# sanderslab/magellanmapper

Measured on AMD Instinct MI355X. Metric: Mvoxels/s, 2048x2048x1024 uint16 stack, 5-sigma LoG blob detection, higher is better.
Workload: dtype f16x2 MFMA (f32 accumulate) + 16-bit fixed-point intermediates; f64 re-score of every candidate

## Files before the change

### magellanmapper_amd/csrc/mmx_rescore.hip

```cpp

#include <algorithm>
#include <type_traits>

#include "mmx_common.h"

#define MMX_MAX_SIGMAS 64

struct mmx_rescore_params {
    int32_t radius[MMX_MAX_SIGMAS];
    double norm[MMX_MAX_SIGMAS];
    int32_t strip;
    int32_t n_blocks;
};

namespace {

template <typename StoreT>
__device__ __forceinline__ double corr_at(const double* vals, int st, int R, const double* w)
{
    double acc = vals[R * st] * w[0];
    for (int k = R; k >= 1; --k) acc += (vals[(R - k) * st] + vals[(R + k) * st]) * w[k];
    return (double)(StoreT)acc;
}

constexpr int kLoadRegs = 16;
constexpr int kMaxCols = 4;
template <typename InT, int NC>
struct z_cfg {
    static constexpr int raw = kLoadRegs / (2 * NC);
    static constexpr int TB = raw >= 8 ? 8 : raw >= 4 ? 4 : raw >= 2 ? 2 : 1;
};
__host__ __device__ __forceinline__ int rescore_col_class(int ncols)
{
    const int cols = (ncols + MMX_WG - 1) / MMX_WG;
    const int passes = (cols + kMaxCols - 1) / kMaxCols;
    const int per = (cols + passes - 1) / passes;
    return per <= 1 ? 1 : per <= 2 ? 2 : 4;
}

template <typename T> struct off_type { using type = T; };

template <typename InT, typename StoreT, int NC, bool INTERIOR, typename OffT>
__device__ __forceinline__ void z_phase(const InT* __restrict__ in, int nyb, int nxb, int pz, int py, int px0, int R, int N,
                                        int SW, int sw, int64_t sz, int64_t sy, int64_t sx,
                                        const int64_t* __restrict__ zr, const double* __restrict__ w0,
                                        const double* __restrict__ w2, double* __restrict__ zp0, double* __restrict__ zp2)
{
    constexpr int TB = z_cfg<InT, NC>::TB;
    const int ncols = N * sw;
    auto zoff = [&](int j) __attribute__((always_inline)) -> int64_t {
        if constexpr (INTERIOR) return (int64_t)(pz + j - R) * sz;
        else return zr[j];
    };
    constexpr bool kBytes = sizeof(OffT) == 4;
    auto ld = [&](OffT o, int64_t z) __attribute__((always_inline)) -> InT {
        if constexpr (kBytes) return *reinterpret_cast<const InT*>(reinterpret_cast<const char*>(in + z) + o);
        else return in[o + z];
    };
    for (int base = 0; base < ncols; base += MMX_WG * NC) {
        OffT off[NC];
        int at[NC];
#pragma unroll
        for (int c = 0; c < NC; ++c) {
            const int e = base + c * MMX_WG + (int)threadIdx.x;
            const int ec = e < ncols ? e : ncols - 1;
            const int dyi = ec / sw;
            const int dxi = ec - dyi * sw;
            const int yy = mmx_reflect(py + dyi - R, nyb);
            const int xx = mmx_reflect(px0 + dxi - R, nxb);
            off[c] = (OffT)(((int64_t)yy * sy + (int64_t)xx * sx) * (kBytes ? (int64_t)sizeof(InT) : 1));
            at[c] = e < ncols ? dyi * SW + dxi : -1;
        }
        double a0[NC], a2[NC];
        {
            const int64_t zc = zoff(R);
            InT ctr[NC];
#pragma unroll
            for (int c = 0; c < NC; ++c) ctr[c] = ld(off[c], zc);
#pragma unroll
            for (int c = 0; c < NC; ++c) {
                const double cv = mmx_vox<InT>::exact(ctr[c]);
                a0[c] = cv * w0[0];
                a2[c] = cv * w2[0];
            }
        }
        int k = R;
        auto batch = [&](auto nb) __attribute__((always_inline)) {
            constexpr int B = decltype(nb)::value;
            for (; k >= B; k -= B) {
                InT lo[NC][B], hi[NC][B];
                if constexpr (kBytes) {
#pragma unroll
                    for (int c = 0; c < NC; ++c) asm volatile("" : "+v"(off[c]));
                }
#pragma unroll
                for (int j = 0; j < B; ++j) {
                    const int64_t zl = zoff(R - (k - j)), zh = zoff(R + (k - j));
#pragma unroll
                    for (int c = 0; c < NC; ++c) {
                        lo[c][j] = ld(off[c], zl);
                        hi[c][j] = ld(off[c], zh);
                    }
                }
#pragma unroll
                for (int c = 0; c < NC; ++c) {
#pragma unroll
                    for (int j = 0; j < B; ++j) {
                        const double p = mmx_vox<InT>::exact(lo[c][j]) + mmx_vox<InT>::exact(hi[c][j]);
                        a0[c] += p * w0[k - j];
                        a2[c] += p * w2[k - j];
                    }
                }
            }
        };
        batch(std::integral_constant<int, TB>{});
        if constexpr (TB > 4) batch(std::integral_constant<int, 4>{});
        if constexpr (TB > 2) batch(std::integral_constant<int, 2>{});
        if constexpr (TB > 1) batch(std::integral_constant<int, 1>{});
#pragma unroll
        for (int c = 0; c < NC; ++c) {
            if (at[c] >= 0) {
                zp0[at[c]] = (double)(StoreT)a0[c];
                zp2[at[c]] = (double)(StoreT)a2[c];
            }
        }
    }
}

template <typename InT, typename StoreT>
__global__ void __launch_bounds__(MMX_WG)
rescore_kernel(const InT* __restrict__ vol, int64_t sz, int64_t sy, int64_t sx,
               const mmx_block* __restrict__ blocks, mmx_cand* __restrict__ pts, uint32_t cap,
               const uint32_t* __restrict__ count, const double* __restrict__ w0_tab,
               const double* __restrict__ w2_tab, mmx_rescore_params prm)
{
    extern __shared__ double smem[];
    uint32_t n = cap;
    if (count) { const uint32_t c = *count; n = c < cap ? c : cap; }
    for (uint64_t idx64 = blockIdx.x; idx64 < n; idx64 += gridDim.x) {
    const uint32_t idx = (uint32_t)idx64;
    const mmx_cand ptv = pts[idx];
    mmx_cand pt;
    pt.slot = __builtin_amdgcn_readfirstlane(ptv.slot);
    pt.s = __builtin_amdgcn_readfirstlane(ptv.s);
    pt.z = __builtin_amdgcn_readfirstlane(ptv.z);
    pt.y = __builtin_amdgcn_readfirstlane(ptv.y);
    pt.x = __builtin_amdgcn_readfirstlane(ptv.x);
    if (pt.slot < 0 || pt.slot >= prm.n_blocks || pt.s < 0 || pt.s >= MMX_MAX_SIGMAS) continue;
    const mmx_block bd = blocks[pt.slot];
    const int R = prm.radius[pt.s];
    const int N = 2 * R + 1;
    const int SW = prm.strip < N ? prm.strip : N;
    const double* w0 = w0_tab + (int64_t)pt.s * (MMX_MAX_RADIUS_GENERIC + 1);
    const double* w2 = w2_tab + (int64_t)pt.s * (MMX_MAX_RADIUS_GENERIC + 1);
    const InT* in = vol + bd.src_off;

    double* zp0 = smem;
    double* zp2 = zp0 + (size_t)N * SW;
    double* yp = zp2 + (size_t)N * SW;
    int64_t* zr = (int64_t*)(yp + 3 * (size_t)N);

    const bool interior = pt.z - R >= 0 && pt.z + R < bd.nz;
    const int cls = rescore_col_class(N * SW);
    const bool small = ((int64_t)(bd.ny - 1) * sy + (int64_t)(bd.nx - 1) * sx) * (int64_t)sizeof(InT) < (1ll << 31)
                       && sy >= 0 && sx >= 0;
    __syncthreads();
    if (!interior) {
        for (int k = threadIdx.x; k < N; k += MMX_WG) zr[k] = (int64_t)mmx_reflect(pt.z + k - R, bd.nz) * sz;
        __syncthreads();
    }
    for (int dx0 = 0; dx0 < N; dx0 += SW) {
        const int sw = (N - dx0) < SW ? (N - dx0) : SW;
        auto zrun = [&](auto nc, auto ot) __attribute__((always_inline)) {
            constexpr int NC = decltype(nc)::value;
            using OffT = typename decltype(ot)::type;
            if (interior)
                z_phase<InT, StoreT, NC, true, OffT>(in, bd.ny, bd.nx, pt.z, pt.y, pt.x + dx0, R, N, SW, sw, sz, sy, sx,
                                                     zr, w0, w2, zp0, zp2);
            else
                z_phase<InT, StoreT, NC, false, OffT>(in, bd.ny, bd.nx, pt.z, pt.y, pt.x + dx0, R, N, SW, sw, sz, sy, sx,
                                                      zr, w0, w2, zp0, zp2);
        };
        if (!small) zrun(std::integral_constant<int, 2>{}, off_type<int64_t>{});
        else switch (cls) {
            case 1: zrun(std::integral_constant<int, 1>{}, off_type<uint32_t>{}); break;
            case 2: zrun(std::integral_constant<int, 2>{}, off_type<uint32_t>{}); break;
            default: zrun(std::integral_constant<int, 4>{}, off_type<uint32_t>{}); break;
        }
        __syncthreads();
        for (int t = threadIdx.x; t < 3 * sw; t += MMX_WG) {
            const int term = t / sw;
            const int dxi = t - term * sw;
            const double* src = (term == 0 ? zp2 : zp0) + dxi;
            yp[term * N + dx0 + dxi] = corr_at<StoreT>(src, SW, R, term == 1 ? w2 : w0);
        }
        __syncthreads();
    }
    if (threadIdx.x < 3)
        zp0[threadIdx.x] = corr_at<StoreT>(yp + threadIdx.x * N, 1, R, threadIdx.x == 2 ? w2 : w0);
    __syncthreads();
    if (threadIdx.x == 0) {
        const StoreT t0 = (StoreT)zp0[0];
        const StoreT t1 = (StoreT)zp0[1];
        const StoreT t2 = (StoreT)zp0[2];
        StoreT sum = t0;
        sum += t1;
        sum += t2;
        const StoreT cube = (-sum) * (StoreT)prm.norm[pt.s];
        pts[idx].v64 = (double)cube;
    }
    }
}

template <typename InT, typename StoreT>
int launch(const mmx_volume* vol, const mmx_block* d_blocks, mmx_cand* d_pts, uint32_t cap,
           const uint32_t* d_count, const double* d_w0, const double* d_w2,
           const mmx_rescore_params& prm, size_t lds, hipStream_t s)
{
    const uint32_t gx = cap < 8192u ? cap : 8192u;
    hipLaunchKernelGGL((rescore_kernel<InT, StoreT>), dim3(gx), dim3(MMX_WG), lds, s,
                       (const InT*)vol->d_data, vol->stride_z, vol->stride_y, vol->stride_x, d_blocks,
                       d_pts, cap, d_count, d_w0, d_w2, prm);
    return hipGetLastError() == hipSuccess ? MMX_OK : MMX_ERR_HIP;
}

}

namespace {
__global__ void __launch_bounds__(MMX_WG)
expand_probes_kernel(mmx_cand* __restrict__ tab, uint32_t cap, uint32_t* __restrict__ count,
                     const uint32_t* __restrict__ n_cands, const mmx_block* __restrict__ blocks, int n_blocks, int ns)
{
    const uint32_t n = *n_cands < cap ? *n_cands : cap;
    for (uint64_t i = (uint64_t)blockIdx.x * MMX_WG + threadIdx.x; i < n; i += (uint64_t)gridDim.x * MMX_WG) {
        const mmx_cand c = tab[i];
        if (!(c.flags & MMX_CAND_CONTESTED) || c.slot < 0 || c.slot >= n_blocks) continue;
        const mmx_block bd = blocks[c.slot];
        const bool banded = (c.flags & MMX_CAND_BAND) != 0;
        int j = 0;
        for (int ds = -1; ds <= 1; ++ds)
            for (int dz = -1; dz <= 1; ++dz)
                for (int dy = -1; dy <= 1; ++dy)
                    for (int dx = -1; dx <= 1; ++dx) {
                        if ((ds | dz | dy | dx) == 0) continue;
                        const int bit = j++;
                        const int ss = c.s + ds, zz = c.z + dz, yy = c.y + dy, xx = c.x + dx;
                        if (ss < 0 || ss >= ns || zz < 0 || zz >= bd.nz || yy < 0 || yy >= bd.ny || xx < 0 || xx >= bd.nx)
                            continue;
                        if (banded && !(bit < 64 ? (c.band >> bit) & 1ull : (c.flags >> (16 + bit - 64)) & 1u)) continue;
                        const uint32_t pos = atomicAdd(count, 1u);
                        if (pos < cap) {
                            mmx_cand r;
                            r.slot = c.slot; r.s = ss; r.z = zz; r.y = yy; r.x = xx;
                            r.flags = MMX_CAND_PROBE;
                            r.v = 0.f; r.nbr_max = 0.f;
                            r.v64 = __longlong_as_double(0x7ff8000000000000LL);
                            r.band = i;
                            tab[pos] = r;
                        }
                    }
    }
}
}

extern "C" int mmx_expand_probes(mmx_cand* d_cands, uint32_t cap, uint32_t* d_count, uint32_t* d_n_cands,
                                 const mmx_block* d_blocks, int n_blocks, int n_sigma, void* stream)
{
    if (!d_cands || !d_count || !d_n_cands || !d_blocks || n_blocks < 1 || n_sigma < 1) return MMX_ERR_ARG;
    hipStream_t s = (hipStream_t)stream;
    if (hipMemcpyAsync(d_n_cands, d_count, sizeof(uint32_t), hipMemcpyDeviceToDevice, s) != hipSuccess) return MMX_ERR_HIP;
    if (cap == 0) return MMX_OK;
    mmx_timed_scope ts(MMX_K_RESCORE, s);
    const uint32_t gx = std::min<uint32_t>(1024u, (cap + MMX_WG - 1) / MMX_WG);
    hipLaunchKernelGGL(expand_probes_kernel, dim3(gx), dim3(MMX_WG), 0, s, d_cands, cap, d_count, d_n_cands, d_blocks,
                       n_blocks, n_sigma);
    return hipGetLastError() == hipSuccess ? MMX_OK : MMX_ERR_HIP;
}

extern "C" int mmx_rescore_f64(const mmx_volume* vol, const mmx_block* d_blocks, int n_blocks,
                               mmx_cand* d_pts, uint32_t cap, const uint32_t* d_count,
                               const double* d_w0, const double* d_w2, const int32_t* h_radius,
                               const double* h_norm, int n_sigma, int store_f32, void* stream)
{
    if (!vol || !vol->d_data || !d_blocks || !d_pts || !d_w0 || !d_w2 || !h_radius || !h_norm)
        return MMX_ERR_ARG;
    if (n_sigma < 1 || n_sigma > MMX_MAX_SIGMAS || n_blocks < 1) return MMX_ERR_ARG;
    if (cap == 0) return MMX_OK;
    mmx_rescore_params prm;
    int rmax = 0;
    for (int i = 0; i < MMX_MAX_SIGMAS; ++i) { prm.radius[i] = 0; prm.norm[i] = 0.0; }
    for (int i = 0; i < n_sigma; ++i) {
        if (h_radius[i] < 0 || h_radius[i] > MMX_MAX_RADIUS_GENERIC) return MMX_ERR_UNSUPPORTED;
        prm.radius[i] = h_radius[i];
        prm.norm[i] = h_norm[i];
        if (h_radius[i] > rmax) rmax = h_radius[i];
    }
    prm.n_blocks = n_blocks;
    const int N = 2 * rmax + 1;
    const size_t budget = 60 * 1024;
    const size_t fixed = (size_t)3 * N * sizeof(double) + (size_t)N * sizeof(int64_t) + 16;
    int strip = (int)((budget - fixed) / ((size_t)2 * N * sizeof(double)));
    if (strip < 1) return MMX_ERR_UNSUPPORTED;
    if (strip > N) strip = N;
    prm.strip = strip;
    const size_t lds = (size_t)2 * N * strip * sizeof(double) + fixed;
    hipStream_t s = (hipStream_t)stream;
    const bool f32s = store_f32 != 0;
    mmx_timed_scope ts(MMX_K_RESCORE, s);
    return mmx_for_voxel<MMX_VOX_ALL>(vol->dtype, MMX_ERR_ARG, [&](auto t) {
        using T = MMX_TAG_T(t);
        if constexpr (std::is_same<T, float>::value)
            if (f32s) return launch<T, float>(vol, d_blocks, d_pts, cap, d_count, d_w0, d_w2, prm, lds, s);
        return launch<T, double>(vol, d_blocks, d_pts, cap, d_count, d_w0, d_w2, prm, lds, s);
    });
}
```

### magellanmapper_amd/csrc/mmx_ymfma.hip

```cpp

#include <type_traits>

#include <cstdlib>

#include "mmx_device.h"

struct ym_cfg {
    float w2[MMX_MAX_RADIUS_FAST + 1];
    float w0[MMX_MAX_RADIUS_FAST + 1];
    float unscale;
    float start;
    float lo, eps;
    int radius;
    int reverse;
};

namespace {

#ifndef YM5_OCC
#define YM5_OCC 2
#endif
#ifndef YM6_WAVES
#define YM6_WAVES 4
#define YM6_JH 4
#define YM6_NF 4
#endif
template <int NB, bool MASK>
__global__ void __launch_bounds__(NB <= 4 ? 256 : YM6_WAVES * 64, NB <= 4 ? 3 : (YM6_WAVES == 4 ? YM5_OCC : 1))
ym_kernel(const mmx_block* __restrict__ blocks, int64_t slot_elems, int64_t tile_stride,
          const unsigned* __restrict__ gt, float* __restrict__ out, ym_cfg cfg,
          unsigned long long* __restrict__ mask)
{
    constexpr int RB = 8 * (NB - 2);
    constexpr int NF = NB <= 4 ? 4 : YM6_NF;
    __shared__ v4u frag[NB * NF * 64];
    constexpr int WAVES = NB <= 4 ? 4 : YM6_WAVES;
    constexpr int JH = NB <= 4 ? 4 : YM6_JH;
    __shared__ float tr[WAVES * 2 * 1024];

    const mmx_block bd = blocks[cfg.reverse ? gridDim.y - 1 - blockIdx.y : blockIdx.y];
    const int ntx = (bd.nx + 15) >> 4, ntz = (bd.nz + 15) >> 4;
    if ((int)blockIdx.x * (WAVES / 4) >= ntx * ntz) return;
    for (int e = threadIdx.x; e < NB * NF * 64; e += WAVES * 64) {
        const int ln = e & 63, f = e >> 6;
        const int piece = (f % NF) % (NF / 2), kern = (f % NF) / (NF / 2), t = f / NF;
        const int m = ln & 15, kq = ln >> 4;
        const int delta = RB - 16 * t;
        unsigned pk[4];
#pragma unroll
        for (int i = 0; i < 8; i += 2) {
            float v[2];
#pragma unroll
            for (int u = 0; u < 2; ++u) {
                int d = 8 * kq + i + u - m + delta;
                d = d < 0 ? -d : d;
                const float ws = d <= cfg.radius ? (kern ? cfg.w0[d] : cfg.w2[d]) : 0.f;
                const float h = (float)(_Float16)ws;
                v[u] = piece == 0 ? h : (piece == 1 ? (ws - h) * 256.f : h * 256.f);
            }
            pk[i >> 1] = pack_h2(v[0], v[1]);
        }
        frag[e] = (v4u){pk[0], pk[1], pk[2], pk[3]};
    }
    __syncthreads();

    const int wv = __builtin_amdgcn_readfirstlane((int)(threadIdx.x >> 6));
    const int tile = (int)blockIdx.x * (WAVES / 4) + (wv >> 2);
    if (tile >= ntx * ntz) return;
    const int c = tile / ntz, U = tile - c * ntz;
    const int zq = wv & 3;
    if (16 * U + 4 * zq >= bd.nz) return;
    const int lane = threadIdx.x & 63;
    const int n = bd.ny;
    const float nms_lo = cfg.lo, nms_eps = cfg.eps, us = cfg.unscale;
    const int kq = lane >> 4, n16 = lane & 15;
    const unsigned trow_b = (unsigned)(ntx * ntz) * 1024u;
    const rsrc_t rs = make_rsrc(gt + (int64_t)bd.slot * tile_stride + (int64_t)tile * 256);
    const unsigned voff = (unsigned)(zq * 256 + n16 * 16);
    const unsigned voff_s = voff + (unsigned)(8 * kq) * trow_b;
    const int xi = lane & 15;
    const int z = 16 * U + 4 * zq + (lane >> 4), x = 16 * c + xi;
    const bool real = z < bd.nz && x < bd.nx;
    float* w1 = out + (int64_t)bd.slot * slot_elems;
    const rsrc_t rsw = make_rsrc(w1);
    const unsigned ooff = (unsigned)((real ? z : 0) * bd.ny * bd.px + (real ? x : 0)) * 4u;
    const unsigned row_b = (unsigned)bd.px * 4u;
    const mmx_entry_geom eg = mmx_entry_geom_make(MMX_MASK_QUADS, bd.nz, bd.nx, bd.px);
    const int nent = eg.per_row;
    ulonglong2* mrow = MASK ? reinterpret_cast<ulonglong2*>(mask) + mmx_entry_base(bd.slot, slot_elems) +
                              mmx_quads_entry(eg, 4 * U + zq, 0) + c
                            : nullptr;
    unsigned long long ab_prev = 0;
    const bool has_l = xi > 0, has_r = xi < 15 && x + 1 < bd.nx;
    float prev1 = -INFINITY, prev2 = -INFINITY, nbx_prev = -INFINITY;
    int ydone = 0;
    float* trw = tr + wv * 2048;

    auto close_pending = [&]() __attribute__((always_inline)) {
        unsigned long long m = 0;
        if (ab_prev) {
            const bool cand = real & (prev1 > nms_lo) & !(fmaxf(prev2, nbx_prev) > prev1 + nms_eps);
            m = __ballot(cand);
        }
        if (lane == 0) *mrow = make_ulonglong2(m, ab_prev);
    };
    auto row = [&](float acc, int y) __attribute__((always_inline)) {
        const unsigned long long ab = MASK ? mmx_above_word(real, acc, nms_lo) : ~0ull;
#ifndef YM_NOSTORE
        if (ab && real) __builtin_amdgcn_raw_buffer_store_b32(__float_as_uint(acc * us), rsw, ooff, (unsigned)y * row_b, 0);
#endif
        if constexpr (MASK) {
            float nbx = -INFINITY;
            if (ab) {
                nbx = mmx_x_neighbours<false>(acc, has_l, has_r);
            }
            if (ydone > 0) {
                unsigned long long m = 0;
                if (ab_prev) {
                    const bool cand = real & (prev1 > nms_lo) & !(fmaxf(fmaxf(prev2, acc), nbx_prev) > prev1 + nms_eps);
                    m = __ballot(cand);
                }
                if (lane == 0) *mrow = make_ulonglong2(m, ab_prev);
                mrow += nent;
            }
            prev2 = prev1; prev1 = acc; nbx_prev = nbx;
            ab_prev = ab;
            ++ydone;
        }
    };
    auto rows_of = [&](int T, int s, bool any) __attribute__((always_inline)) {
        if (T < 0 || 16 * T >= n) return;
        const int cnt = n - 16 * T < 16 ? n - 16 * T : 16;
        if (MASK && !any) {
            if (ydone > 0) {
                close_pending();
                mrow += nent;
            }
            if (lane < cnt - 1) mrow[(int64_t)lane * nent] = make_ulonglong2(0ull, 0ull);
            mrow += (int64_t)(cnt - 1) * nent;
            prev1 = prev2 = nbx_prev = -INFINITY;
            ab_prev = 0;
            ydone += cnt;
            return;
        }
        const float* src = trw + s * 1024 + lane;
        if (!MASK || cnt < 16) {
#pragma unroll 1
            for (int r = 0; r < cnt; ++r) row(src[r * 64], 16 * T + r);
            return;
        }
        float v[16];
#pragma unroll
        for (int r = 0; r < 16; ++r) v[r] = src[r * 64];
        unsigned long long ab[16];
        unsigned long long some = 0;
#pragma unroll
        for (int r = 0; r < 16; ++r) { ab[r] = mmx_above_word(real, v[r], nms_lo); some |= ab[r]; }
        unsigned e0 = 0, e1 = 0, e2 = 0, e3 = 0;
        auto put = [&](int ln, unsigned long long m, unsigned long long a) __attribute__((always_inline)) {
            const bool me = lane == ln;
            e0 = me ? (unsigned)m : e0;
            e1 = me ? (unsigned)(m >> 32) : e1;
            e2 = me ? (unsigned)a : e2;
            e3 = me ? (unsigned)(a >> 32) : e3;
        };
        if (ab_prev) {
            const bool cand = real & (prev1 > nms_lo) & !(fmaxf(fmaxf(prev2, v[0]), nbx_prev) > prev1 + nms_eps);
            put(0, __ballot(cand), ab_prev);
        }
        float nbx15 = -INFINITY;
        if (some) {
#pragma unroll
            for (int r = 0; r < 16; ++r) {
                if (ab[r]) {
#ifndef YM_NOSTORE
                    if (real) __builtin_amdgcn_raw_buffer_store_b32(__float_as_uint(v[r] * us), rsw, ooff, (unsigned)(16 * T + r) * row_b, 0);
#endif
                    const float nbx = mmx_x_neighbours<false>(v[r], has_l, has_r);
                    if (r < 15) {
                        const float below = r > 0 ? v[r > 0 ? r - 1 : 0] : prev1;
                        const bool cand = real & (v[r] > nms_lo) & !(fmaxf(fmaxf(below, v[r < 15 ? r + 1 : 15]), nbx) > v[r] + nms_eps);
                        put(r + 1, __ballot(cand), ab[r]);
                    } else {
                        nbx15 = nbx;
                    }
                }
            }
        }
        if (lane < 16 && (lane > 0 || ydone > 0)) {
            ulonglong2* dst = mrow + (int64_t)(ydone > 0 ? lane : lane - 1) * nent;
            *dst = make_ulonglong2((unsigned long long)e0 | ((unsigned long long)e1 << 32),
                                   (unsigned long long)e2 | ((unsigned long long)e3 << 32));
        }
        mrow += (int64_t)(ydone > 0 ? 16 : 15) * nent;
        prev2 = v[14]; prev1 = v[15]; nbx_prev = nbx15;
        ab_prev = ab[15];
        ydone += 16;
    };

#ifndef YM_PFD
#define YM_PFD 1
#endif
    constexpr int PFD = YM_PFD;
    v4u rawA[8], rawB[PFD == 2 ? 8 : 1];
    auto load_block = [&](int b, v4u (&raw)[8]) __attribute__((always_inline)) {
        const int r0 = -RB + 32 * b;
        if (r0 >= 0 && r0 + 32 <= n) {
#pragma unroll
            for (int i = 0; i < 8; ++i)
                raw[i] = __builtin_bit_cast(v4u, __builtin_amdgcn_raw_buffer_load_b128(rs, voff_s, (unsigned)(r0 + i) * trow_b, 0));
        } else {
#pragma unroll
            for (int i = 0; i < 8; ++i) {
                int v = r0 + 8 * kq + i;
                v = v < 0 ? -1 - v : v;
                v = v >= n ? 2 * n - 1 - v : v;
                v = v < 0 ? 0 : (v > n - 1 ? n - 1 : v);
                raw[i] = __builtin_bit_cast(v4u, __builtin_amdgcn_raw_buffer_load_b128(rs, voff + (unsigned)v * trow_b, 0, 0));
            }
        }
    };
    const int nT = (n + 15) >> 4;
    const int nKB = (nT + NB - 3) / 2 + 1;
    const v4f start = {cfg.start, cfg.start, cfg.start, cfg.start};
    v4f acc[NB][4];
#pragma unroll
    for (int t = 0; t < NB; ++t)
#pragma unroll
        for (int j = 0; j < 4; ++j) acc[t][j] = start;
    bool any0 = false, any1 = false;

    const _Float16 k256 = (_Float16)256.f;
    auto iter = [&](int b, v4u (&raw)[8]) __attribute__((always_inline)) {
#ifndef YM_ROWS_LATE
#define YM_ROWS_LATE 1
#endif
        if (!YM_ROWS_LATE || b == nKB) {
#pragma unroll 1
            for (int h = 0; h < 2; ++h) rows_of(2 * (b - 1) - NB + 2 + h, h, h ? any1 : any0);
        }
        if (b == nKB) return false;
        if constexpr (JH < 4) { any0 = !MASK; any1 = !MASK; }
#pragma unroll
        for (int j0 = 0; j0 < 4; j0 += JH) {
            __builtin_amdgcn_sched_barrier(0);
            v4u pc[JH][4];
#pragma unroll
            for (int j = 0; j < JH; ++j)
#pragma unroll
                for (int p = 0; p < 4; ++p) {
                    const unsigned d0 = raw[2 * p][j0 + j], d1 = raw[2 * p + 1][j0 + j];
                    pc[j][0][p] = __builtin_amdgcn_perm(d1, d0, 0x0c050c01u);
                    pc[j][1][p] = __builtin_amdgcn_perm(d1, d0, 0x0c040c00u);
                    pc[j][2][p] = __builtin_amdgcn_perm(d1, d0, 0x0c070c03u) ^ 0x00800080u;
                    pc[j][3][p] = __builtin_amdgcn_perm(d1, d0, 0x0c060c02u);
                }
            __builtin_amdgcn_sched_barrier(0);
            if (j0 + JH == 4 && b + PFD < nKB) load_block(b + PFD, raw);
            __builtin_amdgcn_sched_barrier(0);
            if (YM_ROWS_LATE && JH == 4) {
#pragma unroll 1
                for (int h = 0; h < 2; ++h) rows_of(2 * (b - 1) - NB + 2 + h, h, h ? any1 : any0);
                __builtin_amdgcn_sched_barrier(0);
            }
            auto tile_mfmas = [&](int t, bool fresh) __attribute__((always_inline)) {
                v4f* a = &acc[t][j0];
                const v4u* fr = frag + (t * NF) * 64 + lane;
                const v4u ah = fr[0], al = fr[64], bh = fr[(NF / 2) * 64], bl = fr[(NF / 2 + 1) * 64];
                const v4u a256 = NF == 6 ? fr[128] : __builtin_bit_cast(v4u, __builtin_bit_cast(v8h, ah) * k256);
                const v4u b256 = NF == 6 ? fr[320] : __builtin_bit_cast(v4u, __builtin_bit_cast(v8h, bh) * k256);
#pragma unroll
                for (int j = 0; j < JH; ++j) a[j] = mfma16(a256, pc[j][0], fresh ? start : a[j]);
#pragma unroll
                for (int j = 0; j < JH; ++j) a[j] = mfma16(ah, pc[j][1], a[j]);
#pragma unroll
                for (int j = 0; j < JH; ++j) a[j] = mfma16(al, pc[j][0], a[j]);
#pragma unroll
                for (int j = 0; j < JH; ++j) a[j] = mfma16(b256, pc[j][2], a[j]);
#pragma unroll
                for (int j = 0; j < JH; ++j) a[j] = mfma16(bh, pc[j][3], a[j]);
#pragma unroll
                for (int j = 0; j < JH; ++j) a[j] = mfma16(bl, pc[j][2], a[j]);
            };
#pragma unroll
            for (int t = 0; t < 2; ++t) tile_mfmas(t, t >= NB - 2);
#pragma unroll
            for (int t = 0; t < 2; ++t) {
                const v4f* a = &acc[t][j0];
                float mx = -INFINITY;
#pragma unroll
                for (int j = 0; j < JH; ++j)
#pragma unroll
                    for (int r = 0; r < 4; ++r) mx = fmaxf(mx, a[j][r]);
                const bool any = MASK ? __ballot(mx > nms_lo) != 0ull : true;
                if constexpr (JH == 4) {
                    if (t == 0) any0 = any; else any1 = any;
                    if (any) {
                        v4f* dst = reinterpret_cast<v4f*>(trw + t * 1024) + (4 * kq) * 16 + n16;
#pragma unroll
                        for (int r = 0; r < 4; ++r) dst[r * 16] = (v4f){a[0][r], a[1][r], a[2][r], a[3][r]};
                    }
                } else {
                    if (t == 0) any0 |= any; else any1 |= any;
                    v2f* dst = reinterpret_cast<v2f*>(trw + t * 1024) + (4 * kq) * 32 + 2 * n16 + (j0 >> 1);
#pragma unroll
                    for (int r = 0; r < 4; ++r) dst[r * 32] = (v2f){a[0][r], a[1][r]};
                }
            }
            __builtin_amdgcn_sched_barrier(0);
#pragma unroll
            for (int t = 2; t < NB; ++t) {
                tile_mfmas(t, t >= NB - 2);
                if constexpr (NB > 4) __builtin_amdgcn_sched_barrier(0);
            }
        }
#pragma unroll
        for (int t = 0; t + 2 < NB; ++t)
#pragma unroll
            for (int j = 0; j < 4; ++j) acc[t][j] = acc[t + 2][j];
        __builtin_amdgcn_wave_barrier();
        return true;
    };
    load_block(0, rawA);
    if constexpr (PFD == 2) {
        if (nKB > 1) load_block(1, reinterpret_cast<v4u (&)[8]>(rawB));
#pragma unroll 1
        for (int b = 0;; b += 2) {
            if (!iter(b, rawA)) break;
            if (!iter(b + 1, reinterpret_cast<v4u (&)[8]>(rawB))) break;
        }
    } else {
#pragma unroll 1
        for (int b = 0; iter(b, rawA); ++b) {}
    }
    if constexpr (MASK) close_pending();
}

template <int NB>
int launch_ym(const mmx_block* d_blocks, int n_blocks, const mmx_zx6_plan& plan, int64_t slot_elems,
              const ym_cfg& cfg, const float* d_p, float* d_log, unsigned long long* d_mask, hipStream_t s)
{
    constexpr int TPW = NB <= 4 ? 1 : YM6_WAVES / 4;
    dim3 grid((plan.max_tiles + TPW - 1) / TPW, n_blocks);
    if (d_mask)
        hipLaunchKernelGGL((ym_kernel<NB, true>), grid, dim3(256 * TPW), 0, s, d_blocks, slot_elems, plan.tile_stride,
                           reinterpret_cast<const unsigned*>(d_p), d_log, cfg, d_mask);
    else
        hipLaunchKernelGGL((ym_kernel<NB, false>), grid, dim3(256 * TPW), 0, s, d_blocks, slot_elems, plan.tile_stride,
                           reinterpret_cast<const unsigned*>(d_p), d_log, cfg, d_mask);
    return hipGetLastError() == hipSuccess ? MMX_OK : MMX_ERR_HIP;
}

}

int mmx_launch_ym(const mmx_block* d_blocks, int n_blocks, const mmx_zx6_plan& plan, int64_t slot_elems,
                  const mmx_taps_f32& taps, int radius, const float* d_p, float cp, float cq, float bias,
                  float* d_log, unsigned long long* d_mask, float nms_lo, float nms_eps, hipStream_t stream)
{
    if (!mmx_ym_accepts(taps.w0, taps.w2, radius, cp, cq)) return MMX_ERR_UNSUPPORTED;
    ym_cfg cfg;
    float mx = 0.f;
    for (int k = 0; k <= radius; ++k) {
        cfg.w2[k] = taps.w2[k] * cp;
        cfg.w0[k] = taps.w0[k] * cq;
        mx = fmaxf(mx, fmaxf(fabsf(cfg.w2[k]), fabsf(cfg.w0[k])));
    }
    int e;
    frexpf(mx, &e);
    const float up = ldexpf(1.f, -e - 1);
    double q128 = 0.0;
    for (int k = 0; k <= MMX_MAX_RADIUS_FAST; ++k) {
        cfg.w2[k] = k <= radius ? cfg.w2[k] * up : 0.f;
        cfg.w0[k] = k <= radius ? cfg.w0[k] * up : 0.f;
        const float h = (float)(_Float16)cfg.w0[k];
        const float l = (float)(_Float16)((cfg.w0[k] - h) * 256.f);
        q128 += (k ? 2.0 : 1.0) * ((double)h * 256.0 + (double)l);
    }
    cfg.unscale = ldexpf(1.f, e + 1 + 24);
    cfg.start = (float)(-128.0 * 0x1p-24 * q128 + (double)bias / (double)cfg.unscale);
    cfg.lo = nms_lo / cfg.unscale;
    cfg.eps = nms_eps / cfg.unscale;
    cfg.radius = radius;
    cfg.reverse = 1;
    if (radius <= 8) return launch_ym<3>(d_blocks, n_blocks, plan, slot_elems, cfg, d_p, d_log, d_mask, stream);
    if (radius <= 16) return launch_ym<4>(d_blocks, n_blocks, plan, slot_elems, cfg, d_p, d_log, d_mask, stream);
    return launch_ym<5>(d_blocks, n_blocks, plan, slot_elems, cfg, d_p, d_log, d_mask, stream);
}
```

Before: 46990.

## Skip dead waves in rescore z-passes and out-of-range MFMA tiles

The rescore z-phase loop moves out to the caller. Each pass now picks its per-thread column count from the columns still left, and each wave picks its own count from its live columns, so fully idle waves skip the loads and FMAs and an NC=3 variant is added. In the y-direction MFMA kernel, tiles whose index falls outside the valid tile range skip their MFMAs and the NMS ballot/store; the accumulators are left undefined through an empty asm. A host helper exposes the pass plan. This removes wasted work at strip and edge boundaries, at the cost of more code variants and the risk that skipped tiles' undefined accumulators leak into later shifts.

```diff
diff --git a/magellanmapper_amd/csrc/mmx_rescore.hip b/magellanmapper_amd/csrc/mmx_rescore.hip
--- a/magellanmapper_amd/csrc/mmx_rescore.hip
+++ b/magellanmapper_amd/csrc/mmx_rescore.hip
@@ -30,19 +30,29 @@
     static constexpr int raw = kLoadRegs / (2 * NC);
     static constexpr int TB = raw >= 8 ? 8 : raw >= 4 ? 4 : raw >= 2 ? 2 : 1;
 };
-__host__ __device__ __forceinline__ int rescore_col_class(int ncols)
-{
-    const int cols = (ncols + MMX_WG - 1) / MMX_WG;
+__host__ __device__ __forceinline__ int rescore_pass_class(int left)
+{
+    const int cols = (left + MMX_WG - 1) / MMX_WG;
     const int passes = (cols + kMaxCols - 1) / kMaxCols;
-    const int per = (cols + passes - 1) / passes;
-    return per <= 1 ? 1 : per <= 2 ? 2 : 4;
+    return (cols + passes - 1) / passes;
+}
+__host__ __forceinline__ int rescore_strip(int rmax, size_t* lds)
+{
+    const int N = 2 * rmax + 1;
+    const size_t budget = 60 * 1024;
+    const size_t fixed = (size_t)3 * N * sizeof(double) + (size_t)N * sizeof(int64_t) + 16;
+    int strip = (int)((budget - fixed) / ((size_t)2 * N * sizeof(double)));
+    if (strip < 1) return 0;
+    if (strip > N) strip = N;
+    if (lds) *lds = (size_t)2 * N * strip * sizeof(double) + fixed;
+    return strip;
 }
 
 template <typename T> struct off_type { using type = T; };
 
 template <typename InT, typename StoreT, int NC, bool INTERIOR, typename OffT>
 __device__ __forceinline__ void z_phase(const InT* __restrict__ in, int nyb, int nxb, int pz, int py, int px0, int R, int N,
-                                        int SW, int sw, int64_t sz, int64_t sy, int64_t sx,
+                                        int SW, int sw, int base, int64_t sz, int64_t sy, int64_t sx,
                                         const int64_t* __restrict__ zr, const double* __restrict__ w0,
                                         const double* __restrict__ w2, double* __restrict__ zp0, double* __restrict__ zp2)
 {
@@ -57,7 +67,7 @@
         if constexpr (kBytes) return *reinterpret_cast<const InT*>(reinterpret_cast<const char*>(in + z) + o);
         else return in[o + z];
     };
-    for (int base = 0; base < ncols; base += MMX_WG * NC) {
+    {
         OffT off[NC];
         int at[NC];
 #pragma unroll
@@ -161,7 +171,7 @@
     int64_t* zr = (int64_t*)(yp + 3 * (size_t)N);
 
     const bool interior = pt.z - R >= 0 && pt.z + R < bd.nz;
-    const int cls = rescore_col_class(N * SW);
+    const int wv = __builtin_amdgcn_readfirstlane((int)(threadIdx.x >> 6));
     const bool small = ((int64_t)(bd.ny - 1) * sy + (int64_t)(bd.nx - 1) * sx) * (int64_t)sizeof(InT) < (1ll << 31)
                        && sy >= 0 && sx >= 0;
     __syncthreads();
@@ -171,21 +181,32 @@
     }
     for (int dx0 = 0; dx0 < N; dx0 += SW) {
         const int sw = (N - dx0) < SW ? (N - dx0) : SW;
-        auto zrun = [&](auto nc, auto ot) __attribute__((always_inline)) {
+        auto zrun = [&](auto nc, auto ot, int base) __attribute__((always_inline)) {
             constexpr int NC = decltype(nc)::value;
             using OffT = typename decltype(ot)::type;
             if (interior)
-                z_phase<InT, StoreT, NC, true, OffT>(in, bd.ny, bd.nx, pt.z, pt.y, pt.x + dx0, R, N, SW, sw, sz, sy, sx,
-                                                     zr, w0, w2, zp0, zp2);
+                z_phase<InT, StoreT, NC, true, OffT>(in, bd.ny, bd.nx, pt.z, pt.y, pt.x + dx0, R, N, SW, sw, base, sz, sy,
+                                                     sx, zr, w0, w2, zp0, zp2);
             else
-                z_phase<InT, StoreT, NC, false, OffT>(in, bd.ny, bd.nx, pt.z, pt.y, pt.x + dx0, R, N, SW, sw, sz, sy, sx,
-                                                      zr, w0, w2, zp0, zp2);
+                z_phase<InT, StoreT, NC, false, OffT>(in, bd.ny, bd.nx, pt.z, pt.y, pt.x + dx0, R, N, SW, sw, base, sz, sy,
+                                                      sx, zr, w0, w2, zp0, zp2);
         };
-        if (!small) zrun(std::integral_constant<int, 2>{}, off_type<int64_t>{});
-        else switch (cls) {
-            case 1: zrun(std::integral_constant<int, 1>{}, off_type<uint32_t>{}); break;
-            case 2: zrun(std::integral_constant<int, 2>{}, off_type<uint32_t>{}); break;
-            default: zrun(std::integral_constant<int, 4>{}, off_type<uint32_t>{}); break;
+        const int ncols = N * sw;
+        for (int base = 0; base < ncols;) {
+            const int nc = small ? rescore_pass_class(ncols - base) : 2;
+            const int mine = ncols - base - 64 * wv;
+            int live = mine <= 0 ? 0 : (mine + MMX_WG - 1) / MMX_WG;
+            live = live < nc ? live : nc;
+            if (!small) {
+                if (live > 0) zrun(std::integral_constant<int, 2>{}, off_type<int64_t>{}, base);
+            } else switch (live) {
+                case 1: zrun(std::integral_constant<int, 1>{}, off_type<uint32_t>{}, base); break;
+                case 2: zrun(std::integral_constant<int, 2>{}, off_type<uint32_t>{}, base); break;
+                case 3: zrun(std::integral_constant<int, 3>{}, off_type<uint32_t>{}, base); break;
+                case 4: zrun(std::integral_constant<int, 4>{}, off_type<uint32_t>{}, base); break;
+                default: break;
+            }
+            base += MMX_WG * nc;
         }
         __syncthreads();
         for (int t = threadIdx.x; t < 3 * sw; t += MMX_WG) {
@@ -277,6 +298,29 @@
     return hipGetLastError() == hipSuccess ? MMX_OK : MMX_ERR_HIP;
 }
 
+extern "C" int mmx_rescore_pass_plan(int radius, int radius_max, int32_t* strip_cols, int32_t* first, int32_t* cols_per_thread,
+                                     int cap)
+{
+    if (radius < 0 || radius > radius_max || radius_max > MMX_MAX_RADIUS_GENERIC || cap < 0) return -1;
+    if (cap > 0 && (!strip_cols || !first || !cols_per_thread)) return -1;
+    const int strip = rescore_strip(radius_max, nullptr);
+    if (strip < 1) return -1;
+    const int N = 2 * radius + 1;
+    const int SW = strip < N ? strip : N;
+    int n = 0;
+    for (int dx0 = 0; dx0 < N; dx0 += SW) {
+        const int sw = (N - dx0) < SW ? (N - dx0) : SW;
+        const int ncols = N * sw;
+        for (int base = 0; base < ncols;) {
+            const int nc = rescore_pass_class(ncols - base);
+            if (n < cap) { strip_cols[n] = ncols; first[n] = base; cols_per_thread[n] = nc; }
+            ++n;
+            base += MMX_WG * nc;
+        }
+    }
+    return n;
+}
+
 extern "C" int mmx_rescore_f64(const mmx_volume* vol, const mmx_block* d_blocks, int n_blocks,
                                mmx_cand* d_pts, uint32_t cap, const uint32_t* d_count,
                                const double* d_w0, const double* d_w2, const int32_t* h_radius,
@@ -296,14 +340,9 @@
         if (h_radius[i] > rmax) rmax = h_radius[i];
     }
     prm.n_blocks = n_blocks;
-    const int N = 2 * rmax + 1;
-    const size_t budget = 60 * 1024;
-    const size_t fixed = (size_t)3 * N * sizeof(double) + (size_t)N * sizeof(int64_t) + 16;
-    int strip = (int)((budget - fixed) / ((size_t)2 * N * sizeof(double)));
-    if (strip < 1) return MMX_ERR_UNSUPPORTED;
-    if (strip > N) strip = N;
-    prm.strip = strip;
-    const size_t lds = (size_t)2 * N * strip * sizeof(double) + fixed;
+    size_t lds = 0;
+    prm.strip = rescore_strip(rmax, &lds);
+    if (prm.strip < 1) return MMX_ERR_UNSUPPORTED;
     hipStream_t s = (hipStream_t)stream;
     const bool f32s = store_f32 != 0;
     mmx_timed_scope ts(MMX_K_RESCORE, s);
diff --git a/magellanmapper_amd/csrc/mmx_ymfma.hip b/magellanmapper_amd/csrc/mmx_ymfma.hip
--- a/magellanmapper_amd/csrc/mmx_ymfma.hip
+++ b/magellanmapper_amd/csrc/mmx_ymfma.hip
@@ -282,10 +282,26 @@
 #pragma unroll
                 for (int j = 0; j < JH; ++j) a[j] = mfma16(bl, pc[j][2], a[j]);
             };
-#pragma unroll
-            for (int t = 0; t < 2; ++t) tile_mfmas(t, t >= NB - 2);
+            auto exists = [&](int t) __attribute__((always_inline)) {
+                if constexpr (NB > 4) return (unsigned)(2 * b - NB + 2 + t) < (unsigned)nT;
+                else return true;
+            };
+            auto run_tile = [&](int t) __attribute__((always_inline)) {
+                if (exists(t)) {
+                    tile_mfmas(t, t >= NB - 2);
+                } else if (t >= NB - 2) {
+#pragma unroll
+                    for (int j = 0; j < JH; ++j) asm volatile("" : "=v"(acc[t][j0 + j]));
+                }
+            };
+#pragma unroll
+            for (int t = 0; t < 2; ++t) run_tile(t);
 #pragma unroll
             for (int t = 0; t < 2; ++t) {
+                if (!exists(t)) {
+                    if constexpr (JH == 4) { if (t == 0) any0 = false; else any1 = false; }
+                    continue;
+                }
                 const v4f* a = &acc[t][j0];
                 float mx = -INFINITY;
 #pragma unroll
@@ -310,7 +326,7 @@
             __builtin_amdgcn_sched_barrier(0);
 #pragma unroll
             for (int t = 2; t < NB; ++t) {
-                tile_mfmas(t, t >= NB - 2);
+                run_tile(t);
                 if constexpr (NB > 4) __builtin_amdgcn_sched_barrier(0);
             }
         }
```

After: 46900. Within noise of the previous version (-0.2%).
